# cvlab-stonybrook/s-volsdf

Hardware: AMD Instinct MI355X
Metric: rendered rays/sec (1024-ray batch, 128 samples) (higher is better)
Workload: dtype f32 (every product, forward and backward, as three fp16 MFMA products of two-piece fp16 operands with f32 accumulate; activation blocks hold both pieces: float32 accuracy class); 1 GPU; configs[1]: VolOpt.train_step (forward + MVS prior lookup + loss + backward + clip/guard/Adam), train mode, fast=1: 1024 rays/GPU x 128 coarse + 98 composited samples + 2048 eikonal points, 8x256 SDF MLP + 4x256 radiance MLP; mode=train, mlp_precision=fp16x2, launch=eager launches, rays_per_gpu=1024, rays_total=1024

## Files before the change

s-volsdf_amd/csrc/svs_mlp_h2_trunk.h:

```cpp
#pragma once
#include "svs_mlp_h2_dev.h"
#include "svs_blocks_h2.h"

namespace svs {
namespace mlp {

struct PosEncBg {
  float v[96];
  __device__ __forceinline__ void compute(float x0, float x1, float x2, float x3) {
    const float xs[4] = {x0, x1, x2, x3};
#pragma unroll
    for (int c = 0; c < 4; ++c) v[c] = xs[c];
#pragma unroll
    for (int f = 0; f < 10; ++f) {
#pragma unroll
      for (int c = 0; c < 4; ++c) {
        float s, co;
        sincosf(xs[c] * (float)(1 << f), &s, &co);
        v[4 + 8 * f + c] = s;
        v[8 + 8 * f + c] = co;
      }
    }
#pragma unroll
    for (int q = 84; q < 96; ++q) v[q] = 0.0f;
  }
};

struct NetFg {
  typedef PosEnc Pe;
  static constexpr int kSteps0 = 3, kPePad = 40, kChunk0 = kChunk0F4, kSpliceTile = 6, kSpliceLocal = 25;
};
struct NetBg {
  typedef PosEncBg Pe;
  static constexpr int kSteps0 = 6, kPePad = 96, kChunk0 = kBgChunk0F4, kSpliceTile = 5, kSpliceLocal = 12;
};

template <bool HBUF, bool LAST, typename Net = NetFg>
struct TrunkEpi {
  static constexpr bool kSplit = !LAST || HBUF;
  f32x16 prev;
  SoftplusA sa;
  float v8[8];
  Pieces2* xn;
  f32x16* y8;
  const typename Net::Pe* pe;
  float* hb;
  int lane, half;
  bool splice;

  __device__ __forceinline__ void a(int r) {
    sa.lg = __builtin_amdgcn_exp2f(__builtin_fabsf(prev[r]) * (-100.0f * 1.44269504088896341f));
    pin(sa.lg);
  }
  __device__ __forceinline__ void a2(int r) {
    asm volatile("v_max_f32 %0, 0, %1" : "=v"(sa.mx) : "v"(prev[r]));
    sa.lg = __builtin_amdgcn_logf(1.0f + sa.lg);
    pin(sa.lg);
  }
  template <bool DEFER = false>
  __device__ __forceinline__ void b(int tp, int r) {
    float v = softplus100_b(sa);
    if (tp == Net::kSpliceTile && splice) {
      constexpr int base = 32 * (7 - Net::kSpliceTile);
      const int l0 = rho(r) - Net::kSpliceLocal, l1 = rho(r) + 4 - Net::kSpliceLocal;
      if (l0 >= 0 || l1 >= 0) {
        const float v0 = l0 >= 0 ? pe->v[base + (l0 >= 0 ? l0 : 0)] : v;
        const float v1 = l1 >= 0 ? pe->v[base + (l1 >= 0 ? l1 : 0)] : v;
        v = half ? v1 : v0;
      }
    }
    pin(v);
    emit<DEFER>(tp, r, v);
  }
  template <bool DEFER = false>
  __device__ __forceinline__ void emit(int tp, int r, float v) {
    if (LAST) y8[tp][r] = v;
    if (kSplit) {
      v8[r & 7] = v;
      if ((r & 7) == 7 && !(DEFER && r == 15)) {
        const int k = 2 * tp + (r >> 3);
        split8(v8, xn->h[k], xn->m[k]);
        pin(xn->h[k], xn->m[k]);
        if (HBUF && !DEFER) { store_piece(hb, k, lane, xn->h[k], 0); store_piece(hb, k, lane, xn->m[k], 1); }
      }
    }
  }
  template <bool STORE = false>
  __device__ __forceinline__ void finish(int tp) {
    if (kSplit) {
      const int k = 2 * tp + 1;
      split8(v8, xn->h[k], xn->m[k]);
      pin(xn->h[k], xn->m[k]);
      if (HBUF && STORE) { store_piece(hb, k, lane, xn->h[k], 0); store_piece(hb, k, lane, xn->m[k], 1); }
    }
  }
  __device__ __forceinline__ void late_store(int t, int s) {
    if (!HBUF) return;
    const int k1 = 2 * (t - 1), k2 = 2 * (t - 2) + 1;
    if (s == 9) store_piece(hb, k1, lane, xn->h[k1], 0);
    if (s == 11) store_piece(hb, k1, lane, xn->m[k1], 1);
    if (t >= 2 && s == 13) store_piece(hb, k2, lane, xn->h[k2], 0);
    if (t >= 2 && s == 15) store_piece(hb, k2, lane, xn->m[k2], 1);
  }
  __device__ __forceinline__ void all(int tp) {
#pragma unroll
    for (int r = 0; r < 16; ++r) { a(r); a2(r); b(tp, r); }
  }
  __device__ __forceinline__ void splice_full_tiles() {
#pragma unroll
    for (int tp = Net::kSpliceTile + 1; tp < 8; ++tp)
#pragma unroll
      for (int r = 0; r < 16; ++r) emit(tp, r, half ? pe->v[32 * (7 - tp) + rho(r) + 4] : pe->v[32 * (7 - tp) + rho(r)]);
  }
};

template <bool HBUF, bool LAST, typename Net = NetFg>
__device__ __forceinline__ void trunk_layer_h2(Stream& st, const Pieces2& x, TrunkEpi<HBUF, LAST, Net>& ep, int lane) {
#pragma unroll
  for (int t = 0; t < 8; ++t) {
    if (t == Net::kSpliceTile + 1 && ep.splice) break;
    f32x16 acc;
    if (t == 0) acc = tile_mma_h2_pf<16, kChunkF4>(st, x, lane, NoEpi(), NoEpi());
    else acc = tile_mma_h2_pf<16, kChunkF4>(st, x, lane, [&](int s) { ep.a(s); }, [&](int s) { ep.a2(s); },
                                            [&](int s) { ep.template b<true>(t - 1, s); ep.late_store(t, s); },
                                            [&]() { if (t >= 2) ep.finish(t - 2); });
    ep.prev = acc;
    if (HBUF && t > 0) { if (t >= 2) st.advance_keep<4>(); else st.advance_keep<2>(); }
    else st.advance();
  }
  if (ep.splice) {
    ep.template finish<true>(Net::kSpliceTile - 1); ep.all(Net::kSpliceTile); ep.splice_full_tiles();
  } else { ep.template finish<true>(6); ep.all(7); }
}

template <bool HBUF, typename Net = NetFg>
__device__ __forceinline__ void forward_trunk_h2(Stream& st, Pieces2& x, Pieces2& xn, f32x16* y8, const typename Net::Pe& pe,
                                                 int lane, int half, float* __restrict__ hbuf) {
  split_pe<Net::kSteps0, Net::kPePad>(pe.v, half, x);
  st.advance();
  {
    TrunkEpi<HBUF, false, Net> ep;
    ep.xn = &xn; ep.y8 = nullptr; ep.pe = &pe; ep.hb = hbuf; ep.lane = lane; ep.half = half; ep.splice = false;
#pragma unroll
    for (int t = 0; t < 8; ++t) {
      if (t < 7) st.prefetch<Net::kChunk0>(); else st.prefetch<kChunkF4>();
      const f32x16 acc = tile_mma_h2<Net::kSteps0>(st.cur_buf(), x, lane);
      if (t > 0) ep.all(t - 1);
      ep.prev = acc;
      st.advance();
    }
    ep.all(7);
  }
  for (int l = 1; l < 7; l += 2) {
    TrunkEpi<HBUF, false, Net> ep;
    ep.y8 = nullptr; ep.pe = &pe; ep.hb = hbuf + (size_t)l * block_stride(); ep.lane = lane; ep.half = half; ep.splice = l == 3;
    ep.xn = &x; trunk_layer_h2<HBUF, false, Net>(st, xn, ep, lane);
    TrunkEpi<HBUF, false, Net> ep2;
    ep2.y8 = nullptr; ep2.pe = &pe; ep2.hb = hbuf + (size_t)(l + 1) * block_stride(); ep2.lane = lane; ep2.half = half; ep2.splice = false;
    ep2.xn = &xn; trunk_layer_h2<HBUF, false, Net>(st, x, ep2, lane);
  }
  TrunkEpi<HBUF, true, Net> ep;
  ep.xn = HBUF ? &x : nullptr; ep.y8 = y8; ep.pe = &pe; ep.hb = hbuf + (size_t)7 * block_stride(); ep.lane = lane; ep.half = half; ep.splice = false;
  trunk_layer_h2<HBUF, true, Net>(st, xn, ep, lane);
}


}
}
```

Before: 299,700 rays/s.

## Carry last-tile softplus epilogue of each trunk layer into next layer's first MFMA tile

The epilogue for the final output tile (tile 7) of each non-last trunk layer is no longer run serially after that layer's MMAs. It is deferred and interleaved into the first tile of the next layer's MFMA loop through carry hooks. The deferred hidden-buffer stores are moved into the following tile as well. This removes an exposed serial block of transcendental and split work between layers, at the cost of carrying one extra epilogue state object, which may raise register pressure, and of more complex store ordering.

```diff
diff --git a/s-volsdf_amd/csrc/svs_mlp_h2_trunk.h b/s-volsdf_amd/csrc/svs_mlp_h2_trunk.h
--- a/s-volsdf_amd/csrc/svs_mlp_h2_trunk.h
+++ b/s-volsdf_amd/csrc/svs_mlp_h2_trunk.h
@@ -57,7 +57,7 @@
     sa.lg = __builtin_amdgcn_logf(1.0f + sa.lg);
     pin(sa.lg);
   }
-  template <bool DEFER = false>
+  template <bool DEFER = false, bool STORE = !DEFER>
   __device__ __forceinline__ void b(int tp, int r) {
     float v = softplus100_b(sa);
     if (tp == Net::kSpliceTile && splice) {
@@ -70,9 +70,9 @@
       }
     }
     pin(v);
-    emit<DEFER>(tp, r, v);
+    emit<DEFER, STORE>(tp, r, v);
   }
-  template <bool DEFER = false>
+  template <bool DEFER = false, bool STORE = !DEFER>
   __device__ __forceinline__ void emit(int tp, int r, float v) {
     if (LAST) y8[tp][r] = v;
     if (kSplit) {
@@ -81,7 +81,7 @@
         const int k = 2 * tp + (r >> 3);
         split8(v8, xn->h[k], xn->m[k]);
         pin(xn->h[k], xn->m[k]);
-        if (HBUF && !DEFER) { store_piece(hb, k, lane, xn->h[k], 0); store_piece(hb, k, lane, xn->m[k], 1); }
+        if (HBUF && STORE) { store_piece(hb, k, lane, xn->h[k], 0); store_piece(hb, k, lane, xn->m[k], 1); }
       }
     }
   }
@@ -102,9 +102,24 @@
     if (t >= 2 && s == 13) store_piece(hb, k2, lane, xn->h[k2], 0);
     if (t >= 2 && s == 15) store_piece(hb, k2, lane, xn->m[k2], 1);
   }
+  template <bool DEFER = false>
   __device__ __forceinline__ void all(int tp) {
 #pragma unroll
-    for (int r = 0; r < 16; ++r) { a(r); a2(r); b(tp, r); }
+    for (int r = 0; r < 16; ++r) { a(r); a2(r); b<DEFER, true>(tp, r); }
+  }
+  __device__ __forceinline__ void carry_a(int s) {
+    if (s == 0) { a(0); a2(0); b(7, 0); }
+    if (s < 15) a(s + 1);
+  }
+  __device__ __forceinline__ void carry_a2(int s) { if (s < 15) a2(s + 1); }
+  __device__ __forceinline__ void carry_b(int s) {
+    if (s < 14) b(7, s + 1);
+    if (s == 14) b<false, false>(7, 15);
+  }
+  __device__ __forceinline__ void carry_store(int s) {
+    if (!HBUF) return;
+    if (s == 13) store_piece(hb, 15, lane, xn->h[15], 0);
+    if (s == 15) store_piece(hb, 15, lane, xn->m[15], 1);
   }
   __device__ __forceinline__ void splice_full_tiles() {
 #pragma unroll
@@ -115,22 +130,27 @@
 };
 
 template <bool HBUF, bool LAST, typename Net = NetFg>
-__device__ __forceinline__ void trunk_layer_h2(Stream& st, const Pieces2& x, TrunkEpi<HBUF, LAST, Net>& ep, int lane) {
+__device__ __forceinline__ void trunk_layer_h2(Stream& st, const Pieces2& x, TrunkEpi<HBUF, LAST, Net>& ep,
+                                               TrunkEpi<HBUF, false, Net>& pc, bool carried, int lane) {
 #pragma unroll
   for (int t = 0; t < 8; ++t) {
     if (t == Net::kSpliceTile + 1 && ep.splice) break;
     f32x16 acc;
-    if (t == 0) acc = tile_mma_h2_pf<16, kChunkF4>(st, x, lane, NoEpi(), NoEpi());
+    if (t == 0) {
+      if (carried) acc = tile_mma_h2_pf<16, kChunkF4>(st, x, lane, [&](int s) { pc.carry_a(s); }, [&](int s) { pc.carry_a2(s); },
+                                                      [&](int s) { pc.carry_b(s); }, [&]() { pc.template finish<true>(6); });
+      else acc = tile_mma_h2_pf<16, kChunkF4>(st, x, lane, NoEpi(), NoEpi());
+    }
     else acc = tile_mma_h2_pf<16, kChunkF4>(st, x, lane, [&](int s) { ep.a(s); }, [&](int s) { ep.a2(s); },
-                                            [&](int s) { ep.template b<true>(t - 1, s); ep.late_store(t, s); },
+                                            [&](int s) { ep.template b<true>(t - 1, s); ep.late_store(t, s); if (t == 1) pc.carry_store(s); },
                                             [&]() { if (t >= 2) ep.finish(t - 2); });
     ep.prev = acc;
-    if (HBUF && t > 0) { if (t >= 2) st.advance_keep<4>(); else st.advance_keep<2>(); }
+    if (HBUF && t > 0) st.advance_keep<4>();
     else st.advance();
   }
   if (ep.splice) {
     ep.template finish<true>(Net::kSpliceTile - 1); ep.all(Net::kSpliceTile); ep.splice_full_tiles();
-  } else { ep.template finish<true>(6); ep.all(7); }
+  } else if (LAST) { ep.template finish<true>(6); ep.all(7); }
 }
 
 template <bool HBUF, typename Net = NetFg>
@@ -138,30 +158,29 @@
                                                  int lane, int half, float* __restrict__ hbuf) {
   split_pe<Net::kSteps0, Net::kPePad>(pe.v, half, x);
   st.advance();
+  TrunkEpi<HBUF, false, Net> epA, epB;
+  epA.y8 = nullptr; epA.pe = &pe; epA.lane = lane; epA.half = half; epA.xn = &x;
+  epB.y8 = nullptr; epB.pe = &pe; epB.lane = lane; epB.half = half; epB.xn = &xn; epB.splice = false;
   {
-    TrunkEpi<HBUF, false, Net> ep;
-    ep.xn = &xn; ep.y8 = nullptr; ep.pe = &pe; ep.hb = hbuf; ep.lane = lane; ep.half = half; ep.splice = false;
+    epB.hb = hbuf;
 #pragma unroll
     for (int t = 0; t < 8; ++t) {
       if (t < 7) st.prefetch<Net::kChunk0>(); else st.prefetch<kChunkF4>();
       const f32x16 acc = tile_mma_h2<Net::kSteps0>(st.cur_buf(), x, lane);
-      if (t > 0) ep.all(t - 1);
-      ep.prev = acc;
+      if (t == 7) epB.template all<true>(6); else if (t > 0) epB.all(t - 1);
+      epB.prev = acc;
       st.advance();
     }
-    ep.all(7);
   }
   for (int l = 1; l < 7; l += 2) {
-    TrunkEpi<HBUF, false, Net> ep;
-    ep.y8 = nullptr; ep.pe = &pe; ep.hb = hbuf + (size_t)l * block_stride(); ep.lane = lane; ep.half = half; ep.splice = l == 3;
-    ep.xn = &x; trunk_layer_h2<HBUF, false, Net>(st, xn, ep, lane);
-    TrunkEpi<HBUF, false, Net> ep2;
-    ep2.y8 = nullptr; ep2.pe = &pe; ep2.hb = hbuf + (size_t)(l + 1) * block_stride(); ep2.lane = lane; ep2.half = half; ep2.splice = false;
-    ep2.xn = &xn; trunk_layer_h2<HBUF, false, Net>(st, x, ep2, lane);
+    epA.hb = hbuf + (size_t)l * block_stride(); epA.splice = l == 3;
+    trunk_layer_h2<HBUF, false, Net>(st, xn, epA, epB, true, lane);
+    epB.hb = hbuf + (size_t)(l + 1) * block_stride();
+    trunk_layer_h2<HBUF, false, Net>(st, x, epB, epA, !epA.splice, lane);
   }
   TrunkEpi<HBUF, true, Net> ep;
   ep.xn = HBUF ? &x : nullptr; ep.y8 = y8; ep.pe = &pe; ep.hb = hbuf + (size_t)7 * block_stride(); ep.lane = lane; ep.half = half; ep.splice = false;
-  trunk_layer_h2<HBUF, true, Net>(st, xn, ep, lane);
+  trunk_layer_h2<HBUF, true, Net>(st, xn, ep, epB, true, lane);
 }
 
 
```

Result: no change. 299,400 rays/s (median of 2 runs) (-0.1%).
